# preon7/2019global

Measured on AMD Instinct MI355X. Metric: Mray/s + ms/frame at 1920x1080, depth 8; %HBM roofline, higher is better.
Workload: dtype f64

## Files before the change

2019global_amd/__init__.py:

```python
from __future__ import annotations

import ctypes
import os
import threading
from typing import Optional, Sequence

import numpy as np

from . import scenes as _scenes

__all__ = [
    "GIError", "lib", "Camera", "Material", "Octree", "ImpSphere", "ImpTriangle", "ExpQuad",
    "ExpSphere", "ExpCube", "ExpCone", "ExpRectangle", "ExpBox",
    "RayTracer", "DeviceScene", "MODE_R", "MODE_X", "STAT_RAYS", "STAT_NODES", "STAT_PRIMS",
    "STAT_PIXELS", "TILE", "MultiScene", "devices_from_env", "obj_entities", "RAY_DOUBLES",
    "AOV_OUTPUTS", "camera_rays", "camera_rays_device",
]

HERE = os.path.dirname(os.path.abspath(__file__))
LIB_PATH = os.environ.get("GI_LIB") or os.path.join(HERE, "libgi.so")

MODE_R, MODE_X = 0, 1
FLAG_STATS = 1
FLAG_R_DFS = 2
FLAG_TIME = 4
FLAG_X_NO_SHADOW = 8
FLAG_X_WF = 16
FLAG_X_MEGA = 32
FLAG_X_SEG = 64
KAT_X_TREE, KAT_X_HBM = 1, 2
X_FORMS = ("k_mode_x", "k_wf_bounce", "k_seg")
R_KERNELS = ("k_mode_r", "k_rf_walk", "k_mode_r_batch")
STAT_RAYS, STAT_NODES, STAT_PRIMS, STAT_PIXELS, STAT_X_PATH_MAX = 0, 1, 2, 3, 4
STAT_X_ITERS, STAT_X_TRAV, STAT_X_HANDLE, STAT_X_HLANES, STAT_X_HCLOSE, STAT_X_HSHADOW = 5, 6, 7, 8, 9, 10
STAT_X_CYC_TRAV, STAT_X_CYC_HIT, STAT_X_CYC_NEXT, STAT_X_CYC_ALL = 11, 12, 13, 14
STAT_X_RESOLVED = 15
STAT_X_IT_NODE, STAT_X_LN_NODE, STAT_X_IT_LEAF, STAT_X_LN_LEAF = 16, 17, 18, 19
STAT_X_IT_RS, STAT_X_LN_RS, STAT_X_IT_ST, STAT_X_LN_ST = 20, 21, 22, 23
STAT_R_PAIRS, STAT_R_OVF_TILES = 24, 25
STATS_N = 26
TILE = 8
ABI_VERSION = 15
RAY_DOUBLES = 8
AOV_OUTPUTS = ("t", "normal", "albedo", "prim", "entity", "uv")
_AOV_KINDS = {"t": (np.float64, ()), "normal": (np.float64, (3,)), "albedo": (np.float64, (3,)),
              "prim": (np.int32, ()), "entity": (np.int32, ()), "uv": (np.int32, (2,))}


class GIError(RuntimeError):
    pass


class EntityDesc(ctypes.Structure):
    _fields_ = [("kind", ctypes.c_int32), ("has_material", ctypes.c_int32), ("args", ctypes.c_double * 11),
                ("mat_color", ctypes.c_double * 3), ("mat_shader", ctypes.c_double * 3),
                ("mat_specular_power", ctypes.c_double), ("mat_reflectivity", ctypes.c_double)]


class SceneDesc(ctypes.Structure):
    _fields_ = [("octree_min", ctypes.c_double * 3), ("octree_max", ctypes.c_double * 3),
                ("n_entities", ctypes.c_int32), ("entities", ctypes.POINTER(EntityDesc))]


class CameraDesc(ctypes.Structure):
    _fields_ = [("pos", ctypes.c_double * 3), ("up", ctypes.c_double * 3), ("forward", ctypes.c_double * 3),
                ("focal", ctypes.c_double)]


class Opts(ctypes.Structure):
    _fields_ = [("mode", ctypes.c_int32), ("spp", ctypes.c_int32), ("depth", ctypes.c_int32),
                ("shard_count", ctypes.c_int32), ("shard_index", ctypes.c_int32), ("band_rows", ctypes.c_int32),
                ("flags", ctypes.c_uint32), ("reserved", ctypes.c_int32), ("seed", ctypes.c_uint64),
                ("stats", ctypes.c_void_p), ("sample_begin", ctypes.c_int32), ("sample_end", ctypes.c_int32)]


class SceneInfo(ctypes.Structure):
    _fields_ = [("n_entities", ctypes.c_int32), ("n_nodes", ctypes.c_int32), ("n_leaves", ctypes.c_int32),
                ("max_depth", ctypes.c_int32), ("n_reachable", ctypes.c_int32), ("n_dropped", ctypes.c_int32),
                ("x_nodes", ctypes.c_int32), ("x_prims", ctypes.c_int32), ("device_bytes", ctypes.c_int64),
                ("x_node_bytes", ctypes.c_int32), ("x_lds_resident", ctypes.c_int32)]


class Hit(ctypes.Structure):
    _fields_ = [("entity", ctypes.c_int32), ("u", ctypes.c_int32), ("v", ctypes.c_int32),
                ("point", ctypes.c_double * 3), ("normal", ctypes.c_double * 3)]


class AovFrame(ctypes.Structure):
    _fields_ = [("w", ctypes.c_int32), ("h", ctypes.c_int32), ("x0", ctypes.c_int32), ("y0", ctypes.c_int32),
                ("x1", ctypes.c_int32), ("y1", ctypes.c_int32)]


class Aov(ctypes.Structure):
    _fields_ = [("t", ctypes.c_void_p), ("normal", ctypes.c_void_p), ("albedo", ctypes.c_void_p),
                ("prim", ctypes.c_void_p), ("entity", ctypes.c_void_p), ("uv", ctypes.c_void_p)]


TILE_CB = ctypes.CFUNCTYPE(None, ctypes.c_void_p, ctypes.c_int, ctypes.c_int, ctypes.POINTER(ctypes.c_uint8),
                           ctypes.POINTER(ctypes.c_double))

EXPORTS = ["gi_abi_version", "gi_last_error", "gi_camera_init", "gi_scene_create", "gi_scene_destroy",
           "gi_scene_get_info", "gi_render", "gi_render_device", "gi_shard_tiles", "gi_unshard_device",
           "gi_trace_ray", "gi_kat_expbox", "gi_kat_x_query", "gi_kat_x_variant", "gi_kat_x_texel", "gi_scene_kernel_ms", "gi_scene_x_form", "gi_scene_seg_ring", "gi_scene_r_kernel", "gi_octree_create", "gi_octree_destroy",
           "gi_octree_intersect", "gi_multi_create", "gi_multi_destroy", "gi_multi_info", "gi_multi_render", "gi_device_count",
           "gi_device_list", "gi_build_id", "gi_obj_parse", "gi_intersect", "gi_occluded", "gi_intersect_device",
           "gi_occluded_device", "gi_render_aov", "gi_render_aov_device", "gi_camera_rays", "gi_camera_rays_device"]

_lib = None
_lock = threading.Lock()


def lib():
    global _lib
# ... 661 lines not shown
```

2019global_amd/build.py:

```python
from __future__ import annotations

import glob
import hashlib
import os
import shutil
import subprocess
import sys

HERE = os.path.dirname(os.path.abspath(__file__))
ROOT = os.path.dirname(HERE)
CSRC = os.path.join(HERE, "csrc")
INCLUDE = os.path.join(ROOT, "include")
OUT = os.path.join(HERE, "libgi.so")
ROCM = os.environ.get("ROCM_PATH", "/opt/rocm")
ARCH = "gfx950"

HOST_SRCS = ["gi_build.cpp", "gi_bvh.cpp", "gi_capi.cpp", "gi_multi.cpp", "gi_obj.cpp"]
DEV_SRCS = ["gi_kernels.hip", "gi_mode_r.hip", "gi_wf.hip"]
HEADERS = ["gi_math.h", "gi_scene.h", "gi_internal.h", "gi_launch.h", "gi_dev.h", "gi_seg_ring.h"]

COMMON = ["-std=c++17", "-fPIC", "-ffp-contract=off", "-fno-fast-math", f"-I{INCLUDE}", f"-I{CSRC}"]


def source_hash() -> str:
    h = hashlib.sha256()
    for name in sorted(HOST_SRCS + DEV_SRCS + HEADERS):
        h.update(name.encode() + b"\0" + open(os.path.join(CSRC, name), "rb").read() + b"\0")
    h.update(b"gi.h\0" + open(os.path.join(INCLUDE, "gi.h"), "rb").read())
    return h.hexdigest()[:16]


def _run(cmd, verbose):
    if verbose:
        print(" ".join(cmd), flush=True)
    subprocess.run(cmd, check=True)


def _stale(out, deps):
    if not os.path.exists(out):
        return True
    t = os.path.getmtime(out)
    return any(os.path.getmtime(d) > t for d in deps)


def build(verbose: bool = False, force: bool = False, variant: str = "", hip_defines=()) -> str:
    hipcc = shutil.which("hipcc") or os.path.join(ROCM, "bin", "hipcc")
    objdir = os.path.join(HERE, "_obj")
    out = OUT
    if variant:
        out = os.path.join(HERE, "_variants", f"libgi_{variant}.so")
        os.makedirs(os.path.dirname(out), exist_ok=True)
    os.makedirs(objdir, exist_ok=True)
# ... 49 lines not shown
```

2019global_amd/csrc/gi_build.cpp:

```cpp
#include <algorithm>
#include <cmath>
#include <cstdlib>
#include <cstring>
#include <string>

#include "gi.h"
#include "gi_scene.h"

namespace gi {

namespace {

struct BEnt {
    REnt rec;
    V3 bmin, bmax;
    std::vector<TriRec> tris;
};

REnt blank_rec(int kind) {
    REnt r;
    memset(&r, 0, sizeof r);
    r.kind = kind;
    r.color[0] = 1; r.color[1] = 0; r.color[2] = 0;
    r.shader[0] = 0.1; r.shader[1] = 0.7; r.shader[2] = 1.0;
    r.spec_pow = 5.0;
    return r;
}

void set_color(REnt& r, const double* c) { r.color[0] = c[0]; r.color[1] = c[1]; r.color[2] = c[2]; }

bool build_entity(const gi_entity_desc& d, BEnt& e, std::string& err) {
    const double* a = d.args;
    switch (d.kind) {
    case GI_IMP_SPHERE: {
        e.rec = blank_rec(K_IMP_SPHERE);
        set_color(e.rec, a + 4);
        e.rec.radius = (float)a[3];
        e.rec.pos[0] = a[0]; e.rec.pos[1] = a[1]; e.rec.pos[2] = a[2];
        const double r = e.rec.radius;
// ... 457 lines not shown
                dev = m;
            }
        }
        if (g < 0) {
            if (groups.size() >= 254) continue;
            groups.push_back(G{n, dot(n, v0)});
            g = (int)groups.size() - 1;
            for (const V3& v : vs) dev = std::max(dev, std::fabs(dot(n, v) - groups[g].off));
        }
        p.pad[0] = g;
        tau = std::max(tau, dev);
        s_min = std::min(s_min, s);
    }
    if (groups.empty()) return;
    for (XWNode& w : hs.xwnodes) {
        uint8_t* b = reinterpret_cast<uint8_t*>(w.pad);
        for (int c = 0; c < 8; ++c) {
            if (w.child[c] >= 0 || w.child[c] == XEMPTY || w.cnt[c] == 0) continue;
            int g = hs.xprims[hs.xhot[~w.child[c]].prim].pad[0];
            for (int j = 1; j < w.cnt[c] && g != kXNoPlane; ++j)
                if (hs.xprims[hs.xhot[~w.child[c] + j].prim].pad[0] != g) g = kXNoPlane;
            b[c] = (uint8_t)g;
        }
    }
    const double K = 2000.0, u = 0x1.0p-53, tmin = 1e-7;
    hs.x_skip_a = K * u / (s_min * tmin);
    hs.x_skip_b = K * (4.0 * u * E / s_min + tau + 4.0 * u * E) / tmin;
}

}

void build_xflat(HostScene& hs) {
    hs.xflat.clear();
    bool ok = true;
    for (const XWNode& w : hs.xwnodes) {
        const uint8_t* g = reinterpret_cast<const uint8_t*>(w.pad);
        for (int c = 0; c < 8; ++c) {
            if (w.child[c] >= 0 || w.child[c] == XEMPTY) continue;
            XFlatLeaf f;
            for (int k = 0; k < 3; ++k) { f.lo[k] = w.lo[k][c]; f.hi[k] = w.hi[k][c]; }
            f.off = ~w.child[c];
            f.cnt = w.cnt[c];
            f.group = g[c];
            f.pad = 0;
            ok = ok && f.cnt <= 255 && f.off < 65536;
            hs.xflat.push_back(f);
        }
    }
    hs.x_flat_ok = ok && hs.xflat.size() <= (size_t)GI_XFLAT_MAX;
}

bool build_host_scene(const gi_scene_desc& desc, HostScene& hs, std::string& err) {
    std::vector<BEnt> ents((size_t)desc.n_entities);
    for (int i = 0; i < desc.n_entities; ++i)
        if (!build_entity(desc.entities[i], ents[i], err)) return false;

    hs.ents.clear();
    hs.tris.clear();
    for (BEnt& e : ents) {
        e.rec.tri_first = (int32_t)hs.tris.size();
        e.rec.tri_count = (int32_t)e.tris.size();
        hs.tris.insert(hs.tris.end(), e.tris.begin(), e.tris.end());
        hs.ents.push_back(e.rec);
    }

    RBuild rb;
    rb.ents = &ents;
    RBuild::N root;
    root.mn = v3(desc.octree_min[0], desc.octree_min[1], desc.octree_min[2]);
    root.mx = v3(desc.octree_max[0], desc.octree_max[1], desc.octree_max[2]);
    rb.nodes.push_back(root);
    hs.n_dropped = 0;
    for (int32_t i = 0; i < desc.n_entities; ++i) {
        if (!bb_overlap(rb.nodes[0].mn, rb.nodes[0].mx, ents[i].bmin, ents[i].bmax)) { ++hs.n_dropped; continue; }
        rb.push_obj(0, i);
    }
    const size_t nn = rb.nodes.size();
    hs.rnodes.assign(nn, RNode());
    hs.leaf_ents.clear();
    std::vector<int32_t> depth(nn, 0);
    std::vector<char> reach((size_t)desc.n_entities, 0);
    hs.n_leaves = 0;
// ... 193 lines not shown
```

2019global_amd/csrc/gi_capi.cpp:

```cpp
#include <hip/hip_runtime_api.h>

#include <algorithm>
#include <cmath>
#include <cstring>
#include <memory>
#include <mutex>
#include <new>
#include <string>
#include <vector>

#include "gi.h"
#include "gi_internal.h"
#include "gi_launch.h"
#include "gi_scene.h"

using namespace gi;

struct HostPath {
    static constexpr int kSlots = 2;
    hipStream_t render = nullptr, copy = nullptr;
    hipEvent_t rendered[kSlots] = {}, copied[kSlots] = {};
    double* d_rgb[kSlots] = {};
    uint8_t* d_rgb8[kSlots] = {};
    double* h_rgb[kSlots] = {};
// ... 402 lines not shown
    const HostScene& h = s->host;
    hipError_t e;
    gi_scene* sp = s.get();
    if ((e = upload(sp, h.rnodes, &d.rnodes)) != hipSuccess || (e = upload(sp, h.leaf_ents, &d.leaf_ents)) != hipSuccess ||
        (e = upload(sp, h.ents, &d.ents)) != hipSuccess || (e = upload(sp, h.tris, &d.tris)) != hipSuccess ||
        (e = upload(sp, h.xwnodes, &d.xwnodes)) != hipSuccess || (e = upload(sp, h.xhot, &d.xhot)) != hipSuccess ||
        (e = upload(sp, h.xbox, &d.xbox)) != hipSuccess ||
        (e = upload(sp, h.xprims, &d.xprims)) != hipSuccess || (e = upload(sp, h.xflat, &d.xflat)) != hipSuccess ||
        (e = upload(sp, std::vector<unsigned>(16, 0u), const_cast<const unsigned**>(&d.work))) != hipSuccess ||
        (e = upload(sp, h.app_off, &d.app_off)) != hipSuccess || (e = upload(sp, h.app_rec, &d.app_rec)) != hipSuccess ||
        (e = upload(sp, h.rpath_rec, &d.rpath_rec)) != hipSuccess || (e = upload(sp, h.rc_nodes, &d.rc_nodes)) != hipSuccess ||
        (e = upload(sp, h.rc_ent, &d.rc_ent)) != hipSuccess || (e = upload(sp, h.rc_maxkey, &d.rc_maxkey)) != hipSuccess ||
        (e = upload(sp, h.r_always, &d.r_always)) != hipSuccess ||
        (e = upload(sp, h.r_leaf_of_rank, &d.r_leaf_of_rank)) != hipSuccess)
        return hip_fail(e, "scene upload");
    d.n_rnodes = (int32_t)h.rnodes.size();
    d.n_ents = (int32_t)h.ents.size();
    d.n_xwnodes = (int32_t)h.xwnodes.size();
    d.n_xprims = (int32_t)h.xprims.size();
    d.x_max_depth = h.x_max_depth;
    d.x_handle8 = h.x_handle8;
    d.x_flags = h.x_flags;
    d.x_skip_a = h.x_skip_a;
    d.x_skip_b = h.x_skip_b;
    d.n_xhot = (int32_t)h.xhot.size();
    d.n_r_always = (int32_t)h.r_always.size();
    d.rc_ext = (float)h.rc_ext;
    {
        const size_t bytes = h.xwnodes.size() * sizeof(XWNode) + h.xhot.size() * sizeof(XHot) +
                             h.xprims.size() * sizeof(XPrim) + h.ents.size() * sizeof(REnt);
        d.x_lds_bytes = bytes <= 40 * 1024 ? (int32_t)bytes : 0;
        d.n_xflat = (int32_t)h.xflat.size();
        d.x_flat = (d.x_lds_bytes > 0 && h.x_flat_ok) ? 1 : 0;
        const size_t per_wg = bytes + 256 * 10 * sizeof(double) + 4 * 68 * sizeof(unsigned);
        d.x_waves4 = (d.x_lds_bytes > 0 && 4 * per_wg <= 160 * 1024) ? 1 : 0;
        d.x_tri_only = 1;
        for (const REnt& r : h.ents)
            if (r.kind == K_IMP_SPHERE || r.kind == K_EXP_SPHERE || r.kind == K_EXP_CONE || r.kind == K_EXP_RECTANGLE) {
                d.x_waves4 = 0;
                d.x_tri_only = 0;
            }
        for (const XPrim& xp : h.xprims)
            if (xp.kind != 0) d.x_tri_only = 0;
        d.r_tri_only = 1;
        for (const REnt& r : h.ents)
            if (r.kind != K_IMP_TRIANGLE) d.r_tri_only = 0;
    }
    const bool want_cn = h.xwnodes.size() * sizeof(XWNode) > (size_t)2 << 20;
    if (d.x_lds_bytes == 0 && want_cn && encode_xcnodes(h.xwnodes, s->host.xcnodes) &&
        (e = upload(sp, h.xcnodes, &d.xcnodes)) != hipSuccess)
        return hip_fail(e, "scene upload (quantised nodes)");
    for (int k = 0; k < 3; ++k) { d.root_lo[k] = INFINITY; d.root_hi[k] = -INFINITY; }
    if (!h.xwnodes.empty())
        for (int c = 0; c < 8; ++c)
            if (h.xwnodes[0].child[c] != XEMPTY)
                for (int k = 0; k < 3; ++k) {
                    d.root_lo[k] = std::min(d.root_lo[k], h.xwnodes[0].lo[k][c]);
                    d.root_hi[k] = std::max(d.root_hi[k], h.xwnodes[0].hi[k][c]);
                }
    d.x_far_r = INFINITY;
    for (int k = 0; k < 3; ++k)
        if (d.root_lo[k] <= d.root_hi[k]) {
            const float m = 16.0f * std::max(std::fabs(d.root_lo[k]), std::fabs(d.root_hi[k]));
            d.x_far_r = std::isinf(d.x_far_r) ? m : std::max(d.x_far_r, m);
        }
    if ((e = x_launch_config(d, device, s->xcfg)) != hipSuccess) return hip_fail(e, "occupancy query");
// ... 55 lines not shown
    out->focal = focal;
    return GI_OK;
}

int gi_scene_create(const gi_scene_desc* desc, gi_scene** out) {
    return guard([&]() -> int {
        if (!desc || !out || desc->n_entities < 0 || (desc->n_entities > 0 && !desc->entities))
            return fail(GI_ERR_ARG, "bad scene descriptor");
        *out = nullptr;
        int ndev = 0;
        hipError_t e = hipGetDeviceCount(&ndev);
        if (e != hipSuccess || ndev <= 0) return fail(GI_ERR_DEVICE, "no HIP device (libgi renders only on gfx950)");
        int dev = 0;
        if ((e = hipGetDevice(&dev)) != hipSuccess) return hip_fail(e, "hipGetDevice");
        return scene_create_on(desc, dev, out);
    });
}

void gi_scene_destroy(gi_scene* s) { destroy_scene(s); }

int gi_scene_get_info(const gi_scene* s, gi_scene_info* info) {
    if (!s || !info) return fail(GI_ERR_ARG, "null argument");
    info->n_entities = (int32_t)s->host.ents.size();
    info->n_nodes = (int32_t)s->host.rnodes.size();
    info->n_leaves = s->host.n_leaves;
    info->max_depth = s->host.max_depth;
    info->n_reachable = s->host.n_reachable;
    info->n_dropped = s->host.n_dropped;
    info->x_nodes = (int32_t)(s->host.xnodes.empty() ? s->host.xwnodes.size() : s->host.xnodes.size());
    info->x_prims = (int32_t)s->host.xprims.size();
    info->device_bytes = s->bytes;
    info->x_node_bytes = s->dev.xcnodes ? (int32_t)sizeof(XCNode) : (int32_t)sizeof(XWNode);
    info->x_lds_resident = s->dev.x_lds_bytes > 0 ? 1 : 0;
    return GI_OK;
}

int64_t gi_shard_tiles(int w, int h, int shard_count) {
    if (w <= 0 || h <= 0 || shard_count < 1) return -1;
    return shard_tiles(w, h, shard_count);
}

int gi_render_device(gi_scene* s, const gi_camera* cam, const double light[3], int w, int h, const gi_opts* o,
                     double* d_rgb, uint8_t* d_rgb8, void* stream) {
    return guard([&]() -> int {
        DeviceRestore keep;
        if (!s) return fail(GI_ERR_ARG, "null scene");
        int rc = check_opts(w, h, o);
        if (rc) return rc;
        if (!cam || !light) return fail(GI_ERR_ARG, "null camera or light");
        std::lock_guard<std::mutex> lk(s->mu);
        if ((rc = prog_check(s, *cam, light, w, h, *o))) return rc;
        rc = scene_render_band(s, make_cam(*cam, w), light, w, h, 0, *o, d_rgb, d_rgb8, static_cast<hipStream_t>(stream),
                               true);
        if (rc == GI_OK) prog_done(s, *o);
        return rc;
    });
}

int gi_render(gi_scene* s, const gi_camera* cam, const double light[3], int w, int h, const gi_opts* o, double* rgb,
              uint8_t* rgb8, const volatile int* cancel, gi_tile_cb cb, void* user) {
    return guard([&]() -> int {
        DeviceRestore keep;
        if (!s) return fail(GI_ERR_ARG, "null scene");
        int rc = check_opts(w, h, o);
        if (rc) return rc;
        if (!cam || !light) return fail(GI_ERR_ARG, "null camera or light");
// ... 480 lines not shown
```

2019global_amd/csrc/gi_kernels.hip:

```cpp
#include <hip/hip_runtime.h>

#include <algorithm>
#include <cfloat>
#include <cmath>
#include <cstdlib>
#include <mutex>

#include "gi.h"
#include "gi_dev.h"
#include "gi_launch.h"
#include "gi_scene.h"

namespace gi {

namespace {

enum : int { PH_CLOSEST = 0, PH_SHADOW = 1, PH_NEED = 2, PH_START = 3, PH_DEAD = 4, PH_DONEPX = 5, PH_HELP = 6 };

#ifndef GI_X_START_BURST
#define GI_X_START_BURST 16
#endif
#ifndef GI_X_MIN_WAVES
#define GI_X_MIN_WAVES 3
#endif
// ... 685 lines not shown
    const double n = (double)wk.s1;
    const double c0 = smin(a / n, 1.0), c1 = smin(b / n, 1.0), c2 = smin(c / n, 1.0);
    if (rgb) { rgb[3 * idx] = c0; rgb[3 * idx + 1] = c1; rgb[3 * idx + 2] = c2; }
    if (rgb8) quantize(c0, c1, c2, rgb8 + 3 * idx);
}

__global__ __launch_bounds__(256) void k_unshard(TileMap m, const double* packed, const uint8_t* packed8, double* rgb,
                                                  uint8_t* rgb8) {
    const long long i = (long long)blockIdx.x * blockDim.x + threadIdx.x;
    const long long t = i / (kTile * kTile);
    if (t >= m.n_tiles) return;
    const int lane = (int)(i % (kTile * kTile));
    const int ty = (int)(t / m.tiles_x), tx = (int)(t % m.tiles_x);
    const int x = tx * kTile + (lane & 7), y = ty * kTile + (lane >> 3);
    if (x >= m.w || y >= m.h) return;
    const long long r = t % m.shard_count, lt = t / m.shard_count;
    const long long src = (r * m.n_local + lt) * (kTile * kTile) + lane;
    const long long dst = (long long)y * m.w + x;
    if (rgb) { rgb[3 * dst] = packed[3 * src]; rgb[3 * dst + 1] = packed[3 * src + 1]; rgb[3 * dst + 2] = packed[3 * src + 2]; }
    if (rgb8) { rgb8[3 * dst] = packed8[3 * src]; rgb8[3 * dst + 1] = packed8[3 * src + 1]; rgb8[3 * dst + 2] = packed8[3 * src + 2]; }
}


}

long long shard_tiles(int w, int h, int shard_count) { return make_map(w, h, shard_count, 0).n_local; }

const XEnv& x_env() {
    static XEnv env;
    static std::once_flag once;
    std::call_once(once, [] {
        if (const char* v = std::getenv("GI_X_HELP")) env.help = std::atoi(v) != 0;
        if (const char* v = std::getenv("GI_X_FLAT")) env.flat = std::atoi(v) != 0;
        if (const char* v = std::getenv("GI_SEG_RING")) env.seg_ring = std::atoi(v) != 0;
        if (const char* v = std::getenv("GI_R_FLAT")) env.r_flat = std::atoi(v);
        if (const char* v = std::getenv("GI_RF_PER_SLOT")) env.rf_per_slot = std::max(0, std::min(1024, std::atoi(v)));
        if (const char* v = std::getenv("GI_X_WF")) env.wf = std::atoi(v);
        if (const char* v = std::getenv("GI_RF_GROUP")) env.rf_group = (std::atoi(v) == 1 || std::atoi(v) == 4) ? std::atoi(v) : 0;
        const char* v = std::getenv("GI_X_MAX_RUN");
        const int r = v ? std::max(1, std::min(128, std::atoi(v))) : GI_X_MAX_RUN;
        int lg = 0;
        while ((2 << lg) <= r) ++lg;
        env.run_log2 = lg;
    });
    return env;
}

#ifndef GI_WF_MAX_DEPTH
#define GI_WF_MAX_DEPTH 64
#endif
XForm x_form_choice(const DevScene& sc, const XLaunchCfg& xc, const gi_opts& o) {
    if (o.mode != GI_MODE_X || (o.flags & GI_FLAG_X_MEGA)) return XFORM_MEGA;
    if (o.flags & GI_FLAG_X_SEG) return XFORM_SEG;
    const XForm wf = o.depth <= GI_WF_MAX_DEPTH ? XFORM_WF : XFORM_MEGA;
    if (o.flags & GI_FLAG_X_WF) return wf;
    const XEnv& env = x_env();
    if (env.wf >= 0) return env.wf == XFORM_WF ? wf : env.wf == XFORM_SEG ? XFORM_SEG : XFORM_MEGA;
    return (xc.var.lds || (size_t)sc.n_xwnodes * sizeof(XWNode) <= ((size_t)1 << 20)) ? XFORM_SEG : XFORM_MEGA;
}

namespace {
template <typename F>
void x_dispatch(const DevScene& sc, bool help, bool stats, F&& f) {
    with_bools([&](auto S, auto HP, auto C, auto H, auto T) { f(&k_mode_x<S.value, HP.value, C.value, H.value, T.value>); },
               stats, help, sc.xcnodes != nullptr, sc.x_max_depth <= 7, sc.x_tri_only != 0);
}
// ... 106 lines not shown
```

2019global_amd/csrc/gi_launch.h:

```cpp
#pragma once

#include <hip/hip_runtime_api.h>

#include "gi.h"
#include "gi_scene.h"

namespace gi {

struct XEnv {
    int run_log2 = 0, help = 1, wf = -1, flat = 1, seg_ring = 1;
    int r_flat = -1;
    int rf_per_slot = 16;
    int rf_group = 0;
};
const XEnv& x_env();

struct XKernelCfg {
    XVariant var;
    bool flat;
    size_t lds_bytes;
    int resident;
};

long long shard_tiles(int w, int h, int shard_count);
constexpr long long kXWfChunk = 8ll << 20;
hipError_t x_launch_config(const DevScene& sc, int device, XLaunchCfg& cfg);
XForm x_form_choice(const DevScene& sc, const XLaunchCfg& xc, const gi_opts& o);
hipError_t launch_render(const DevScene& sc, const XLaunchCfg& xc, const CamDev& cam, V3 light, int w, int h, int y0,
                         const gi_opts& o, double* rgb, uint8_t* rgb8, const XScratch& xs, KTimer* kt,
                         hipStream_t stream);
hipError_t launch_unshard(int w, int h, int shard_count, const double* packed, const uint8_t* packed8, double* rgb,
                          uint8_t* rgb8, hipStream_t stream);

RKernel r_kernel_choice(const DevScene& sc, const gi_opts& o);
unsigned rf_own_pairs();
unsigned rf_page_pairs();
unsigned rf_max_pages();
unsigned rf_seg_pairs();
hipError_t launch_mode_r(const DevScene& sc, const CamDev& cam, V3 light, int w, int h, int y0, const gi_opts& o,
                         double* rgb, uint8_t* rgb8, const XScratch& xs, hipStream_t stream, hipEvent_t ev_begin,
                         hipEvent_t ev_end);
hipError_t launch_trace_ray(const DevScene& sc, V3 o, V3 d, V3 light, int32_t* out_i, double* out_d, hipStream_t stream);
hipError_t launch_box_kat(int n, const double* recs, int32_t* out, hipStream_t stream);
// ... 19 lines not shown
```

2019global_amd/csrc/gi_scene.h:

```cpp
#pragma once
#include <stdint.h>
#include <string>
#include <type_traits>
#include <vector>

#include "gi.h"
#include "gi_math.h"

namespace gi {

struct CamDev {
    V3 pos, up, left, top_left;
    double rx, ry;
};

enum EntKind : int32_t { K_IMP_SPHERE = 1, K_IMP_TRIANGLE = 2, K_EXP_QUAD = 3, K_EXP_SPHERE = 4, K_EXP_CUBE = 5,
                         K_EXP_CONE = 6, K_EXP_RECTANGLE = 7, K_EXP_BOX = 8 };

struct RNode {
    double mn[3], mx[3];
    int32_t child0;
    int32_t parent;
    int32_t ent_off;
    int32_t ent_cnt;
// ... 64 lines not shown
    uint8_t qlo[3][8];
    uint8_t qhi[3][8];
    int32_t child[8];
    uint8_t cnt[8];
    int32_t parent;
    int32_t pad[5];
};
static_assert(sizeof(XCNode) == 128, "XCNode layout");
bool encode_xcnodes(const std::vector<XWNode>& w, std::vector<XCNode>& out);

struct XHot {
    double a[3], b[3], c[3];
    int32_t prim;
    int32_t kind;
};
static_assert(sizeof(XHot) == 80, "XHot layout");
struct XBox {
    float lo[3], hi[3];
    int32_t pad[2];
};
static_assert(sizeof(XBox) == 32, "XBox layout");
struct XLeaf {
    int32_t off, cnt;
};
#ifndef GI_XFLAT_MAX
#define GI_XFLAT_MAX 32
#endif
static_assert(GI_XFLAT_MAX >= 1 && GI_XFLAT_MAX <= 32, "the candidate mask is one 32-bit word");
struct XFlatLeaf {
    float lo[3], hi[3];
    int32_t off;
    uint16_t cnt;
    uint8_t group;
    uint8_t pad;
};
static_assert(sizeof(XFlatLeaf) == 32, "XFlatLeaf layout");

struct HostScene {
    std::vector<RNode> rnodes;
    std::vector<int32_t> leaf_ents;
    std::vector<REnt> ents;
    std::vector<TriRec> tris;
    int32_t max_depth = 0, n_leaves = 0, n_reachable = 0, n_dropped = 0;
    std::vector<XNode> xnodes;
    std::vector<XWNode> xwnodes;
    std::vector<XCNode> xcnodes;
    std::vector<XLeaf> xleaves;
    std::vector<int32_t> xprim_idx;
    std::vector<XHot> xhot;
    std::vector<XBox> xbox;
    std::vector<XPrim> xprims;
    int32_t x_max_depth = 0;
    std::vector<int32_t> app_off;
    std::vector<int32_t> app_leaf;
    std::vector<int64_t> app_rank;
    std::vector<int32_t> rpath_off;
    std::vector<int32_t> rpath;
    std::vector<RPathRec> rpath_rec;
    std::vector<RApp> app_rec;
    std::vector<XWNode> rc_nodes;
    std::vector<int32_t> rc_ent;
    std::vector<int64_t> rc_maxkey;
    std::vector<int32_t> r_always;
    std::vector<int32_t> r_leaf_of_rank;
    double rc_ext = 0;
    int32_t x_handle8 = 6;
    int32_t x_flags = 0;
    double x_est_nodes = 0, x_est_prims = 0;
    bool x_spatial = false;
    double x_skip_a = 0.0, x_skip_b = 2.0;
    std::vector<XFlatLeaf> xflat;
    bool x_flat_ok = false;
};
bool build_host_scene(const gi_scene_desc& desc, HostScene& hs, std::string& err);
void build_xflat(HostScene& hs);

inline void finalize_xwnodes(std::vector<XWNode>& w) {
    for (XWNode& n : w) {
        n.exists = 0;
        for (int c = 0; c < 8; ++c)
            if (n.child[c] != XEMPTY) n.exists |= 1 << c;
    }
}

void build_xbvh(const std::vector<XPrim>& prims, const std::vector<double>& bounds, int leaf_max, HostScene& hs,
                bool geometric = false);
void build_rcand(HostScene& hs);

struct DevScene {
    const RNode* rnodes;
    const int32_t* leaf_ents;
    const REnt* ents;
    const TriRec* tris;
    const XWNode* xwnodes;
    const XCNode* xcnodes;
    const XHot* xhot;
    const XBox* xbox;
    const XPrim* xprims;
    unsigned* work;
    int32_t n_rnodes, n_ents, n_xwnodes, n_xprims;
    int32_t x_max_depth;
    int32_t x_handle8;
    int32_t x_flags;
    int32_t n_xhot;
    int32_t x_lds_bytes;
    int32_t x_waves4;
    int32_t x_tri_only;
    int32_t r_tri_only;
    float root_lo[3], root_hi[3];
    double x_skip_a, x_skip_b;
    const int32_t* app_off;
    const RApp* app_rec;
    const RPathRec* rpath_rec;
    const XWNode* rc_nodes;
    const int32_t* rc_ent;
    const int64_t* rc_maxkey;
    const int32_t* r_always;
    const int32_t* r_leaf_of_rank;
    int32_t n_r_always;
    float rc_ext;
    const XFlatLeaf* xflat;
    int32_t n_xflat;
    int32_t x_flat;
    float x_far_r;
};

struct KTimer {
    static constexpr int kRing = 64;
    void* ev0[kRing] = {};
    void* ev1[kRing] = {};
    long long recorded = 0;
    double sum_ms = 0.0;
    long long folded = 0;
};

struct XScratch {
    unsigned* list = nullptr;
    double* part = nullptr;
    long long cap = 0;
    int spp = 0;
    double* wq[2] = {nullptr, nullptr};
    unsigned* wid[2] = {nullptr, nullptr};
    unsigned* wcnt = nullptr;
    long long wcap = 0;
    unsigned* rf_pairs = nullptr;
    unsigned* rf_pt = nullptr;
    unsigned long long* rf_best = nullptr;
    double* rf_dir = nullptr;
    unsigned* rf_cnt = nullptr;
    unsigned* rf_ovf = nullptr;
    unsigned* rf_rcnt = nullptr;
    unsigned* rf_soff = nullptr;
    unsigned* rf_shc = nullptr;
    unsigned* rf_sreg = nullptr;
    unsigned* rf_hoff = nullptr;
    unsigned rf_pages = 0;
    long long rf_slots = 0;
    size_t rf_bytes = 0;
// ... 69 lines not shown
```

2019global_amd/csrc/gi_wf.hip:

```cpp
#include <hip/hip_runtime.h>

#include <algorithm>
#include <cstdlib>
#include <mutex>
#include <type_traits>

#include "gi.h"
#include "gi_dev.h"
#include "gi_launch.h"
#include "gi_scene.h"
#include "gi_seg_ring.h"

namespace gi {
namespace {

constexpr long long kWfTile = 8;

#ifndef GI_WF_MIN_WAVES_LDS
#define GI_WF_MIN_WAVES_LDS 4
#endif
#ifndef GI_WF_MIN_WAVES
#define GI_WF_MIN_WAVES 3
#endif
#ifndef GI_WF_TAKE
#define GI_WF_TAKE 16
#endif
constexpr size_t kWfSlotBytes = 8 * 256 * sizeof(double);
constexpr int kSegRingPlanes = 5;
constexpr size_t kSegRingBytes = 4 * kSegRingPlanes * kSegBatch * sizeof(uint64_t);
constexpr int kSegPlaneBits = 8, kSegPlaneMask = (1 << kSegPlaneBits) - 1;

struct PathId {
    uint64_t key;
    unsigned smp;
    int b;
};
__device__ __forceinline__ void slot_put_u64(double* pl, int f, uint64_t v) { reinterpret_cast<uint64_t*>(pl)[f * 256] = v; }
__device__ __forceinline__ uint64_t slot_get_u64(const double* pl, int f) { return reinterpret_cast<const uint64_t*>(pl)[f * 256]; }

struct WFQ {
    double* r;
// ... 118 lines not shown
    return *(const __attribute__((address_space(4))) u32x8*)(uintptr_t)(tab + k);
}
__device__ __forceinline__ uint32_t flat_pack(uint32_t off, int k, uint32_t w7) { return off | ((uint32_t)k << 16) | ((w7 & 0xFFu) << 24); }
__device__ __forceinline__ uint32_t flat_shift_in(uint32_t m, unsigned long long hm) {
    uint32_t r;
    asm("v_addc_co_u32 %0, vcc, %1, %1, %2" : "=v"(r) : "v"(m), "s"(hm) : "vcc");
    return r;
}
__device__ __forceinline__ int flat_key(float tn, int k) {
    int r;
    asm("v_bfi_b32 %0, 31, %1, %2" : "=v"(r) : "s"(k), "v"(tn));
    return r;
}
__device__ __forceinline__ int flat_med3(int a, int b, int c) { return max(min(a, b), min(max(a, b), c)); }
__device__ __forceinline__ float flat_key_floor(int e) { return __int_as_float(e & ~31); }
__device__ __forceinline__ uint32_t flat_pk_of(const uint32_t* pkw, int k) { return pkw[k]; }
__device__ __forceinline__ bool flat_hit(const XFlatLeaf* r, F3 no, F3 ivf, int sm, float tmax, uint32_t& pk, int k) {
    const int4* q = reinterpret_cast<const int4*>(r);
    const int4 a = q[0], b = q[1];
    const float lx = __int_as_float(a.x), ly = __int_as_float(a.y), lz = __int_as_float(a.z);
    const float hx = __int_as_float(a.w), hy = __int_as_float(b.x), hz = __int_as_float(b.y);
    const float nx = (sm & 1) ? hx : lx, fx = (sm & 1) ? lx : hx;
    const float ny = (sm & 2) ? hy : ly, fy = (sm & 2) ? ly : hy;
    const float nz = (sm & 4) ? hz : lz, fz = (sm & 4) ? lz : hz;
    const float tn = fmaxf(fmaxf(__builtin_fmaf(nx, ivf.x, no.x), __builtin_fmaf(ny, ivf.y, no.y)),
                           fmaxf(__builtin_fmaf(nz, ivf.z, no.z), 0.0f));
    const float tf = fminf(fminf(__builtin_fmaf(fx, ivf.x, no.x), __builtin_fmaf(fy, ivf.y, no.y)),
                           fminf(__builtin_fmaf(fz, ivf.z, no.z), tmax));
    pk = flat_pack((uint32_t)b.z, k, (uint32_t)b.w);
    return tn <= tf;
}
template <bool ANY, bool TRI>
__device__ __forceinline__ int wf_flat(float far_r, const XFlatLeaf* tab, const uint32_t* pkw, int n, const XHot* H, V3 o, V3 d, double tmax, bool act,
                                       double& t_out, uint32_t& nnode, uint32_t& nprim, uint32_t& nsteps, int skip) {
    const F3 of = ray_org32(o, d, far_r);
    const F3 ivf = inv_dir(d);
    const F3 no = neg_oiv(of, ivf);
    const int sm = iv_signs(ivf);
    const bool sx = (sm & 1) != 0, sy = (sm & 2) != 0, sz = (sm & 4) != 0;
    double tb = tmax;
    float tbf = up32(tmax);
    int best = -1;
    const float tfa = __builtin_canonicalizef(act ? tbf : -1.0f);
    constexpr int kNone = 0x7F800000;
    uint32_t m = 0, pk = 0;
    int e1 = kNone, e2 = kNone;
    auto step = [&](const u32x8 w, int k) {
        const float lx = __uint_as_float(w[0]), ly = __uint_as_float(w[1]), lz = __uint_as_float(w[2]);
        const float hx = __uint_as_float(w[3]), hy = __uint_as_float(w[4]), hz = __uint_as_float(w[5]);
        const float ax = __builtin_fmaf(lx, ivf.x, no.x), bx = __builtin_fmaf(hx, ivf.x, no.x);
        const float ay = __builtin_fmaf(ly, ivf.y, no.y), by = __builtin_fmaf(hy, ivf.y, no.y);
        const float az = __builtin_fmaf(lz, ivf.z, no.z), bz = __builtin_fmaf(hz, ivf.z, no.z);
        const float tn = fmaxf(fmaxf(sx ? bx : ax, sy ? by : ay), fmaxf(sz ? bz : az, 0.0f));
        const float tf = fminf(fminf(sx ? ax : bx, sy ? ay : by), fminf(sz ? az : bz, tfa));
        const bool in = tn <= tf, other = (int)((w[7] >> 16) & 0xFFu) != skip;
        m = flat_shift_in(m, __builtin_amdgcn_ballot_w64(in) & __builtin_amdgcn_ballot_w64(other));
        if (!ANY) {
            const int key = flat_key(tn, k);
            const int eh = (in & other) ? key : kNone;
            e2 = flat_med3(e1, e2, eh);
            e1 = min(e1, eh);
        }
    };
    int k0 = 0;
    for (; k0 + 4 <= n; k0 += 4) {
        const u32x8 w0 = flat_rec_uniform(tab, k0), w1 = flat_rec_uniform(tab, k0 + 1);
        const u32x8 w2 = flat_rec_uniform(tab, k0 + 2), w3 = flat_rec_uniform(tab, k0 + 3);
        step(w0, k0);
        step(w1, k0 + 1);
        step(w2, k0 + 2);
        step(w3, k0 + 3);
    }
#pragma unroll 1
    for (int k = k0; k < n; ++k) step(flat_rec_uniform(tab, k), k);
    if (act) nnode += (uint32_t)((n * (int)sizeof(XFlatLeaf) + 255) / 256);
    bool go = m != 0;
    if (go) {
        const int bit = (ANY || e1 == kNone) ? __builtin_ctz(m) : n - 1 - (e1 & 31);
        m &= ~(1u << bit);
        pk = flat_pk_of(pkw, n - 1 - bit);
    }
    while (go) {
        ++nsteps;
        const int cnt = (int)(pk >> 24);
        const XHot* hp = H + (pk & 0xFFFFu);
        for (int j = 0; j < cnt; j += 2) {
            const bool two = j + 1 < cnt;
            const XHotR r0 = load_hot(hp + j), r1 = load_hot(hp + (two ? j + 1 : j));
            const double ta = x_prim_t<TRI>(r0.h, o, d, MX_TMIN);
            const double tq = two ? x_prim_t<TRI>(r1.h, o, d, MX_TMIN) : INFINITY;
            nprim += two ? 2 : 1;
            if (ANY) {
                if ((ta < tmax) | (tq < tmax)) {
                    best = ta < tmax ? r0.h.prim : r1.h.prim;
                    break;
                }
            } else {
                const bool ua = (ta < tb) | ((ta == tb) & (r0.h.prim < best));
                tb = ua ? ta : tb;
                best = ua ? r0.h.prim : best;
                const bool uq = (tq < tb) | ((tq == tb) & (r1.h.prim < best));
                tb = uq ? tq : tb;
                best = uq ? r1.h.prim : best;
                tbf = up32(tb);
            }
        }
        go = false;
        if (ANY) {
            if (best < 0 && m != 0) {
                const int bit = __builtin_ctz(m);
                m &= m - 1;
                pk = flat_pk_of(pkw, n - 1 - bit);
                go = true;
            }
        } else {
            if (flat_key_floor(e2) > tbf) m = 0;
            while (m != 0) {
                const int bit = 31 - __builtin_clz(m);
// ... 83 lines not shown
    }
    return primary_dir(cam, (double)x + jx, (double)y + jy);
}
__device__ __forceinline__ bool wf_primary_misses(const DevScene& sc, const CamDev& cam, V3 d0) {
    const F3 iv0 = f3(__builtin_amdgcn_rcpf((float)d0.x), __builtin_amdgcn_rcpf((float)d0.y), __builtin_amdgcn_rcpf((float)d0.z));
    return !root_hit(sc, ray_org32(cam.pos, d0, ray_far_r(sc, cam.pos)), iv0);
}
__device__ __forceinline__ void wf_store(double* part, double* rgb, uint8_t* rgb8, int spp, long long idx, unsigned smp, V3 L) {
    if (spp > 1) {
        double* q = part + 3 * ((size_t)idx * (size_t)spp + (size_t)smp);
        q[0] = L.x; q[1] = L.y; q[2] = L.z;
    } else {
        const double c0 = smin((0.0 + L.x) / 1.0, 1.0), c1 = smin((0.0 + L.y) / 1.0, 1.0), c2 = smin((0.0 + L.z) / 1.0, 1.0);
        if (rgb) { rgb[3 * idx] = c0; rgb[3 * idx + 1] = c1; rgb[3 * idx + 2] = c2; }
        if (rgb8) quantize(c0, c1, c2, rgb8 + 3 * idx);
    }
}

struct WFSegStats {
    uint64_t it_c = 0, ln_c = 0, it_s = 0, ln_s = 0, segs = 0, live = 0, iters = 0;
    uint64_t cyc_c = 0, cyc_s = 0, cyc_sh = 0, cyc_ref = 0, cyc_all = 0;
};
__device__ __forceinline__ void wf_wave_steps(uint32_t n, uint64_t& it, uint64_t& ln) {
    uint32_t mx = n, sm = n;
    for (int off = 32; off > 0; off >>= 1) {
        mx = max(mx, (uint32_t)__shfl_xor(mx, off));
        sm += __shfl_xor(sm, off);
    }
    if ((threadIdx.x & 63) == 0) { it += mx; ln += sm; }
}
template <bool ANY, bool LDS, bool SH, bool TRI, bool CN, bool FLAT>
__device__ __forceinline__ int x_query(const DevScene& sc, const WFView& v, float far_r, const V3& o, const V3& d, double tmax,
                                       bool act, double& t_out, uint32_t& nnode, uint32_t& nprim, uint32_t& st_steps, int skip) {
    if constexpr (FLAT) return wf_flat<ANY, TRI>(far_r, v.FT, v.FP, sc.n_xflat, v.LH, o, d, tmax, act, t_out, nnode, nprim, st_steps, skip);
    else if constexpr (LDS) return wf_trace<ANY, true, false, SH, TRI, false>(far_r, v.LW, v.LH, o, d, tmax, act, v.nst, t_out, nnode, nprim, st_steps, skip);
    else if constexpr (CN) return wf_trace<ANY, false, false, SH, TRI, true>(far_r, sc.xcnodes, sc.xhot, o, d, tmax, act, v.nst, t_out, nnode, nprim, st_steps);
    else return wf_trace<ANY, false, false, SH, TRI, true>(far_r, sc.xwnodes, sc.xhot, o, d, tmax, act, v.nst, t_out, nnode, nprim, st_steps, skip);
}
__device__ __forceinline__ int x_own_plane(int pg, const V3& pn, const V3& dir, double skip_cos) {
    return (pg < 254 && fabs(dot(dir, pn)) >= skip_cos) ? pg : 254;
}
struct XHitFrame { V3 P, Ld, pn; double ldist; int pg; };
__device__ __forceinline__ XHitFrame x_hit_frame(const WFView& v, const V3& light, const V3& o, const V3& d, bool hit, int best, double t) {
    XHitFrame h{o, v3(0, 0, 1), v3(0, 0, 1), 0.0, 254};
    if (hit) {
        h.P = o + t * d;
        const V3 lv = light - h.P;
        h.ldist = gsqrt(dot(lv, lv));
        h.Ld = normalize(lv);
        const XPrim& px = v.XP[best];
        h.pg = px.pad[0] < 254 ? px.pad[0] : 254;
        h.pn = ld3(px.n);
    }
    return h;
}

template <bool STATS, bool LDS, bool SH, bool TRI, bool CN, bool FLAT, typename KeyF>
__device__ __forceinline__ bool x_segment(const DevScene& sc, const WFView& v, const V3& light, int depth, bool no_shadow, bool act,
                                          const KeyF& id_of, V3& o, V3& d, V3& L, V3& T,
                                          uint32_t& nnode, uint32_t& nprim, uint32_t& nrays, WFSegStats& ws,
                                          double skip_cos = 2.0, int* splane = nullptr, float far_r = INFINITY) {
    uint32_t st_steps = 0;
    uint64_t c0 = STATS ? clock64() : 0;
    bool occl = false;
    double tbest = INFINITY;
    const int skip_c = splane ? (*splane & kSegPlaneMask) : 254;
    const int best = x_query<false, LDS, SH, TRI, CN, FLAT>(sc, v, far_r, o, d, INFINITY, act, tbest, nnode, nprim, st_steps, skip_c);
// ... 771 lines not shown
```

include/gi.h:

```cpp
#ifndef GI_H_
#define GI_H_

#include <stddef.h>
#include <stdint.h>

#ifdef __cplusplus
extern "C" {
#endif

#define GI_ABI_VERSION 15

typedef enum gi_status {
    GI_OK = 0,
    GI_ERR_ARG = -1,
    GI_ERR_DEVICE = -2,
    GI_ERR_SCENE = -3,
    GI_ERR_CANCELLED = -4,
    GI_ERR_NOMEM = -5,
    GI_ERR_INTERNAL = -6
} gi_status;

typedef enum gi_entity_kind {
    GI_IMP_SPHERE = 1,
    GI_IMP_TRIANGLE = 2,
    GI_EXP_QUAD = 3,
    GI_EXP_SPHERE = 4,
    GI_EXP_CUBE = 5,
    GI_EXP_CONE = 6,
    GI_EXP_RECTANGLE = 7,
    GI_EXP_BOX = 8
} gi_entity_kind;

typedef struct gi_entity_desc {
    int32_t kind;
    int32_t has_material;
    double args[11];
    double mat_color[3];
    double mat_shader[3];
    double mat_specular_power;
    double mat_reflectivity;
} gi_entity_desc;

typedef struct gi_scene_desc {
// ... 52 lines not shown
#define GI_STAT_X_CYC_TRAV 11
#define GI_STAT_X_CYC_HIT 12
#define GI_STAT_X_CYC_NEXT 13
#define GI_STAT_X_CYC_ALL 14
#define GI_STAT_X_RESOLVED 15
#define GI_STAT_X_IT_NODE 16
#define GI_STAT_X_LN_NODE 17
#define GI_STAT_X_IT_LEAF 18
#define GI_STAT_X_LN_LEAF 19
#define GI_STAT_X_IT_RS 20
#define GI_STAT_X_LN_RS 21
#define GI_STAT_X_IT_ST 22
#define GI_STAT_X_LN_ST 23
#define GI_STAT_R_PAIRS 24
#define GI_STAT_R_OVF_TILES 25
#define GI_STATS_N 26

#define GI_TILE 8

typedef struct gi_scene gi_scene;

typedef struct gi_scene_info {
    int32_t n_entities;
    int32_t n_nodes;
    int32_t n_leaves;
    int32_t max_depth;
    int32_t n_reachable;
    int32_t n_dropped;
    int32_t x_nodes;
    int32_t x_prims;
    int64_t device_bytes;
    int32_t x_node_bytes;
    int32_t x_lds_resident;
} gi_scene_info;

typedef struct gi_hit {
    int32_t entity;
    int32_t u, v;
    double point[3], normal[3];
} gi_hit;

typedef void (*gi_tile_cb)(void* user, int y0, int rows, const uint8_t* rgb8_rows, const double* rgb_rows);

int gi_abi_version(void);
const char* gi_last_error(void);
int gi_device_count(void);
int gi_device_list(int32_t* out, int cap);
const char* gi_build_id(void);

int gi_camera_init(const double pos[3], const double look_at[3], double focal, gi_camera* out);

int gi_scene_create(const gi_scene_desc* desc, gi_scene** out);
void gi_scene_destroy(gi_scene* scene);
int gi_scene_get_info(const gi_scene* scene, gi_scene_info* info);

int gi_render(gi_scene* scene, const gi_camera* cam, const double light[3], int w, int h,
              const gi_opts* opts, double* rgb, uint8_t* rgb8, const volatile int* cancel,
              gi_tile_cb cb, void* user);

int gi_render_device(gi_scene* scene, const gi_camera* cam, const double light[3], int w, int h,
                     const gi_opts* opts, double* d_rgb, uint8_t* d_rgb8, void* stream);

int64_t gi_shard_tiles(int w, int h, int shard_count);

int gi_unshard_device(int w, int h, int shard_count, const double* d_packed, const uint8_t* d_packed8,
                      double* d_rgb, uint8_t* d_rgb8, void* stream);
// ... 55 lines not shown
```

Measured before the change: 36240.

## Test only one triangle of coplanar fan-pair quad leaves in flat traversal

Adds a build-time check that marks two-triangle leaves forming a coplanar, convex fan pair sharing a diagonal. In the flat LDS traversal, a cheap edge-side test on the shared diagonal chooses which triangle the ray can hit, so normally only one triangle intersection runs. When the choice is numerically unsure, the lane also tests the second triangle, guarded by a wave ballot. It is enabled only when every flat leaf qualifies, and it adds branch divergence and extra code in the hot loop.

Result: faster. 37110 (median of 6 runs) (+2.4%).

```diff
diff --git a/2019global_amd/__init__.py b/2019global_amd/__init__.py
--- a/2019global_amd/__init__.py
+++ b/2019global_amd/__init__.py
@@ -40,7 +40,7 @@
 STAT_R_PAIRS, STAT_R_OVF_TILES = 24, 25
 STATS_N = 26
 TILE = 8
-ABI_VERSION = 15
+ABI_VERSION = 16
 RAY_DOUBLES = 8
 AOV_OUTPUTS = ("t", "normal", "albedo", "prim", "entity", "uv")
 _AOV_KINDS = {"t": (np.float64, ()), "normal": (np.float64, (3,)), "albedo": (np.float64, (3,)),
@@ -78,7 +78,8 @@
     _fields_ = [("n_entities", ctypes.c_int32), ("n_nodes", ctypes.c_int32), ("n_leaves", ctypes.c_int32),
                 ("max_depth", ctypes.c_int32), ("n_reachable", ctypes.c_int32), ("n_dropped", ctypes.c_int32),
                 ("x_nodes", ctypes.c_int32), ("x_prims", ctypes.c_int32), ("device_bytes", ctypes.c_int64),
-                ("x_node_bytes", ctypes.c_int32), ("x_lds_resident", ctypes.c_int32)]
+                ("x_node_bytes", ctypes.c_int32), ("x_lds_resident", ctypes.c_int32),
+                ("x_flat_leaves", ctypes.c_int32), ("x_fan_leaves", ctypes.c_int32)]
 
 
 class Hit(ctypes.Structure):
diff --git a/2019global_amd/build.py b/2019global_amd/build.py
--- a/2019global_amd/build.py
+++ b/2019global_amd/build.py
@@ -17,7 +17,7 @@
 
 HOST_SRCS = ["gi_build.cpp", "gi_bvh.cpp", "gi_capi.cpp", "gi_multi.cpp", "gi_obj.cpp"]
 DEV_SRCS = ["gi_kernels.hip", "gi_mode_r.hip", "gi_wf.hip"]
-HEADERS = ["gi_math.h", "gi_scene.h", "gi_internal.h", "gi_launch.h", "gi_dev.h", "gi_seg_ring.h"]
+HEADERS = ["gi_math.h", "gi_scene.h", "gi_internal.h", "gi_launch.h", "gi_dev.h", "gi_seg_ring.h", "gi_fan_pair.h"]
 
 COMMON = ["-std=c++17", "-fPIC", "-ffp-contract=off", "-fno-fast-math", f"-I{INCLUDE}", f"-I{CSRC}"]
 
diff --git a/2019global_amd/csrc/gi_build.cpp b/2019global_amd/csrc/gi_build.cpp
--- a/2019global_amd/csrc/gi_build.cpp
+++ b/2019global_amd/csrc/gi_build.cpp
@@ -5,6 +5,7 @@
 #include <string>
 
 #include "gi.h"
+#include "gi_fan_pair.h"
 #include "gi_scene.h"
 
 namespace gi {
@@ -528,6 +529,7 @@
 
 void build_xflat(HostScene& hs) {
     hs.xflat.clear();
+    hs.n_fan_leaves = 0;
     bool ok = true;
     for (const XWNode& w : hs.xwnodes) {
         const uint8_t* g = reinterpret_cast<const uint8_t*>(w.pad);
@@ -538,12 +540,14 @@
             f.off = ~w.child[c];
             f.cnt = w.cnt[c];
             f.group = g[c];
-            f.pad = 0;
+            f.fan = (f.cnt == 2 && fan_pair_ok(hs.xhot[(size_t)f.off], hs.xhot[(size_t)f.off + 1])) ? 1 : 0;
+            hs.n_fan_leaves += f.fan;
             ok = ok && f.cnt <= 255 && f.off < 65536;
             hs.xflat.push_back(f);
         }
     }
     hs.x_flat_ok = ok && hs.xflat.size() <= (size_t)GI_XFLAT_MAX;
+    hs.x_fan_all = !hs.xflat.empty() && (size_t)hs.n_fan_leaves == hs.xflat.size();
 }
 
 bool build_host_scene(const gi_scene_desc& desc, HostScene& hs, std::string& err) {
diff --git a/2019global_amd/csrc/gi_capi.cpp b/2019global_amd/csrc/gi_capi.cpp
--- a/2019global_amd/csrc/gi_capi.cpp
+++ b/2019global_amd/csrc/gi_capi.cpp
@@ -458,6 +458,7 @@
         d.x_lds_bytes = bytes <= 40 * 1024 ? (int32_t)bytes : 0;
         d.n_xflat = (int32_t)h.xflat.size();
         d.x_flat = (d.x_lds_bytes > 0 && h.x_flat_ok) ? 1 : 0;
+        d.x_fan = (d.x_flat && h.x_fan_all && x_env().fan) ? 1 : 0;
         const size_t per_wg = bytes + 256 * 10 * sizeof(double) + 4 * 68 * sizeof(unsigned);
         d.x_waves4 = (d.x_lds_bytes > 0 && 4 * per_wg <= 160 * 1024) ? 1 : 0;
         d.x_tri_only = 1;
@@ -579,6 +580,8 @@
     info->device_bytes = s->bytes;
     info->x_node_bytes = s->dev.xcnodes ? (int32_t)sizeof(XCNode) : (int32_t)sizeof(XWNode);
     info->x_lds_resident = s->dev.x_lds_bytes > 0 ? 1 : 0;
+    info->x_flat_leaves = (int32_t)s->host.xflat.size();
+    info->x_fan_leaves = s->host.n_fan_leaves;
     return GI_OK;
 }
 
diff --git a/2019global_amd/csrc/gi_fan_pair.h b/2019global_amd/csrc/gi_fan_pair.h
--- /dev/null
+++ b/2019global_amd/csrc/gi_fan_pair.h
@@ -0,0 +1,54 @@
+#ifndef GI_FAN_PAIR_H_
+#define GI_FAN_PAIR_H_
+
+#include "gi_math.h"
+#include "gi_scene.h"
+
+namespace gi {
+
+constexpr double kFanParTol = 0x1.0p-44;
+constexpr double kFanSliver = 0x1.0p-6;
+constexpr double kFanMargin = 0x1.0p-24;
+constexpr double kFanFloor = 0x1.0p-960;
+
+enum FanChoice : int { FAN_T1 = 0, FAN_T2 = 1, FAN_BOTH = 2 };
+
+GI_HD double fan_abs(double x) { return __builtin_fabs(x); }
+GI_HD double fan_n1(V3 v) { return fan_abs(v.x) + fan_abs(v.y) + fan_abs(v.z); }
+GI_HD bool fan_same_bits(const double* p, const double* q) {
+    return mx_f64_to_bits(p[0]) == mx_f64_to_bits(q[0]) && mx_f64_to_bits(p[1]) == mx_f64_to_bits(q[1]) &&
+           mx_f64_to_bits(p[2]) == mx_f64_to_bits(q[2]);
+}
+
+GI_HD bool fan_pair_ok(const XHot& r0, const XHot& r1) {
+    if (r0.kind != 0 || r1.kind != 0) return false;
+    if (!fan_same_bits(r0.a, r1.a) || !fan_same_bits(r0.c, r1.b)) return false;
+    const V3 e1 = ld3(r0.b), D = ld3(r0.c), e2 = ld3(r1.c);
+    const V3 n1 = cross(e1, D), n2 = cross(D, e2);
+    const double s1 = fan_n1(n1), s2 = fan_n1(n2);
+    if (!(s1 >= kFanSliver * (fan_n1(e1) * fan_n1(D))) || !(s2 >= kFanSliver * (fan_n1(D) * fan_n1(e2)))) return false;
+    if (!(s1 > 0.0) || !(s2 > 0.0) || !(s1 * s2 < INFINITY)) return false;
+    if (!(dot(n1, n2) > 0.0)) return false;
+    const V3 x = cross(n1, n2);
+    const double tol = kFanParTol * (s1 * s2);
+    if (!(fan_abs(x.x) <= tol) || !(fan_abs(x.y) <= tol) || !(fan_abs(x.z) <= tol)) return false;
+    const V3 nb = cross(D - e1, e2 - e1), nd = cross(e1, e2);
+    return dot(nb, n1) > 0.0 && dot(nd, n1) > 0.0;
+}
+
+GI_HD int fan_pair_choice(const XHot& r0, V3 o, V3 d) {
+    const V3 e1 = ld3(r0.b), D = ld3(r0.c), v0 = ld3(r0.a);
+    const V3 pv = fcross(d, D);
+    const double det = fdot(e1, pv);
+    const V3 tv = o - v0;
+    const double un = fdot(tv, pv);
+    const bool pos = det > 0.0;
+    const bool t1_miss = (pos & (un < 0.0)) | (!pos & (un > 0.0));
+    const double k = (kFanMargin * fan_n1(d)) * fan_n1(D);
+    const bool sure = (fan_abs(un) > gfma(k, fan_n1(tv), kFanFloor)) & (fan_abs(det) > gfma(k, fan_n1(e1), kFanFloor));
+    return t1_miss ? FAN_T2 : (sure ? FAN_T1 : FAN_BOTH);
+}
+
+}
+
+#endif
diff --git a/2019global_amd/csrc/gi_kernels.hip b/2019global_amd/csrc/gi_kernels.hip
--- a/2019global_amd/csrc/gi_kernels.hip
+++ b/2019global_amd/csrc/gi_kernels.hip
@@ -741,6 +741,7 @@
     std::call_once(once, [] {
         if (const char* v = std::getenv("GI_X_HELP")) env.help = std::atoi(v) != 0;
         if (const char* v = std::getenv("GI_X_FLAT")) env.flat = std::atoi(v) != 0;
+        if (const char* v = std::getenv("GI_X_FAN")) env.fan = std::atoi(v) != 0;
         if (const char* v = std::getenv("GI_SEG_RING")) env.seg_ring = std::atoi(v) != 0;
         if (const char* v = std::getenv("GI_R_FLAT")) env.r_flat = std::atoi(v);
         if (const char* v = std::getenv("GI_RF_PER_SLOT")) env.rf_per_slot = std::max(0, std::min(1024, std::atoi(v)));
diff --git a/2019global_amd/csrc/gi_launch.h b/2019global_amd/csrc/gi_launch.h
--- a/2019global_amd/csrc/gi_launch.h
+++ b/2019global_amd/csrc/gi_launch.h
@@ -8,7 +8,7 @@
 namespace gi {
 
 struct XEnv {
-    int run_log2 = 0, help = 1, wf = -1, flat = 1, seg_ring = 1;
+    int run_log2 = 0, help = 1, wf = -1, flat = 1, seg_ring = 1, fan = 1;
     int r_flat = -1;
     int rf_per_slot = 16;
     int rf_group = 0;
diff --git a/2019global_amd/csrc/gi_scene.h b/2019global_amd/csrc/gi_scene.h
--- a/2019global_amd/csrc/gi_scene.h
+++ b/2019global_amd/csrc/gi_scene.h
@@ -120,7 +120,7 @@
     int32_t off;
     uint16_t cnt;
     uint8_t group;
-    uint8_t pad;
+    uint8_t fan;
 };
 static_assert(sizeof(XFlatLeaf) == 32, "XFlatLeaf layout");
 
@@ -159,6 +159,8 @@
     double x_skip_a = 0.0, x_skip_b = 2.0;
     std::vector<XFlatLeaf> xflat;
     bool x_flat_ok = false;
+    int32_t n_fan_leaves = 0;
+    bool x_fan_all = false;
 };
 bool build_host_scene(const gi_scene_desc& desc, HostScene& hs, std::string& err);
 void build_xflat(HostScene& hs);
@@ -211,7 +213,9 @@
     int32_t n_xflat;
     int32_t x_flat;
     float x_far_r;
-};
+    int32_t x_fan;
+};
+static_assert(sizeof(DevScene) == 264, "DevScene layout");
 
 struct KTimer {
     static constexpr int kRing = 64;
diff --git a/2019global_amd/csrc/gi_wf.hip b/2019global_amd/csrc/gi_wf.hip
--- a/2019global_amd/csrc/gi_wf.hip
+++ b/2019global_amd/csrc/gi_wf.hip
@@ -7,6 +7,7 @@
 
 #include "gi.h"
 #include "gi_dev.h"
+#include "gi_fan_pair.h"
 #include "gi_launch.h"
 #include "gi_scene.h"
 #include "gi_seg_ring.h"
@@ -191,7 +192,7 @@
 }
 template <bool ANY, bool TRI>
 __device__ __forceinline__ int wf_flat(float far_r, const XFlatLeaf* tab, const uint32_t* pkw, int n, const XHot* H, V3 o, V3 d, double tmax, bool act,
-                                       double& t_out, uint32_t& nnode, uint32_t& nprim, uint32_t& nsteps, int skip) {
+                                       double& t_out, uint32_t& nnode, uint32_t& nprim, uint32_t& nsteps, int skip, bool fan) {
     const F3 of = ray_org32(o, d, far_r);
     const F3 ivf = inv_dir(d);
     const F3 no = neg_oiv(of, ivf);
@@ -243,6 +244,33 @@
         ++nsteps;
         const int cnt = (int)(pk >> 24);
         const XHot* hp = H + (pk & 0xFFFFu);
+        if (TRI && fan) {
+            const XHotR r0 = load_hot(hp);
+            const int ch = fan_pair_choice(r0.h, o, d);
+            const XHotR rc = load_hot(hp + (ch == FAN_T2 ? 1 : 0));
+            const double ta = x_prim_t<TRI>(rc.h, o, d, MX_TMIN);
+            double tq = INFINITY;
+            int pq = rc.h.prim;
+            if (__builtin_amdgcn_ballot_w64(ch == FAN_BOTH) != 0) {
+                if (ch == FAN_BOTH) {
+                    const XHotR r1 = load_hot(hp + 1);
+                    tq = x_prim_t<TRI>(r1.h, o, d, MX_TMIN);
+                    pq = r1.h.prim;
+                }
+            }
+            nprim += 2;
+            if (ANY) {
+                if ((ta < tmax) | (tq < tmax)) best = ta < tmax ? rc.h.prim : pq;
+            } else {
+                const bool ua = (ta < tb) | ((ta == tb) & (rc.h.prim < best));
+                tb = ua ? ta : tb;
+                best = ua ? rc.h.prim : best;
+                const bool uq = (tq < tb) | ((tq == tb) & (pq < best));
+                tb = uq ? tq : tb;
+                best = uq ? pq : best;
+                tbf = up32(tb);
+            }
+        } else
         for (int j = 0; j < cnt; j += 2) {
             const bool two = j + 1 < cnt;
             const XHotR r0 = load_hot(hp + j), r1 = load_hot(hp + (two ? j + 1 : j));
@@ -392,7 +420,7 @@
 template <bool ANY, bool LDS, bool SH, bool TRI, bool CN, bool FLAT>
 __device__ __forceinline__ int x_query(const DevScene& sc, const WFView& v, float far_r, const V3& o, const V3& d, double tmax,
                                        bool act, double& t_out, uint32_t& nnode, uint32_t& nprim, uint32_t& st_steps, int skip) {
-    if constexpr (FLAT) return wf_flat<ANY, TRI>(far_r, v.FT, v.FP, sc.n_xflat, v.LH, o, d, tmax, act, t_out, nnode, nprim, st_steps, skip);
+    if constexpr (FLAT) return wf_flat<ANY, TRI>(far_r, v.FT, v.FP, sc.n_xflat, v.LH, o, d, tmax, act, t_out, nnode, nprim, st_steps, skip, sc.x_fan != 0);
     else if constexpr (LDS) return wf_trace<ANY, true, false, SH, TRI, false>(far_r, v.LW, v.LH, o, d, tmax, act, v.nst, t_out, nnode, nprim, st_steps, skip);
     else if constexpr (CN) return wf_trace<ANY, false, false, SH, TRI, true>(far_r, sc.xcnodes, sc.xhot, o, d, tmax, act, v.nst, t_out, nnode, nprim, st_steps);
     else return wf_trace<ANY, false, false, SH, TRI, true>(far_r, sc.xwnodes, sc.xhot, o, d, tmax, act, v.nst, t_out, nnode, nprim, st_steps, skip);
diff --git a/include/gi.h b/include/gi.h
--- a/include/gi.h
+++ b/include/gi.h
@@ -8,7 +8,7 @@
 extern "C" {
 #endif
 
-#define GI_ABI_VERSION 15
+#define GI_ABI_VERSION 16
 
 typedef enum gi_status {
     GI_OK = 0,
@@ -127,6 +127,8 @@
     int64_t device_bytes;
     int32_t x_node_bytes;
     int32_t x_lds_resident;
+    int32_t x_flat_leaves;
+    int32_t x_fan_leaves;
 } gi_scene_info;
 
 typedef struct gi_hit {
```
